# zdebruine/RcppML

Hardware: AMD Instinct MI355X
Metric: ALS updates/sec (cols solved/s), k=64 sparse NMF (higher is better)
Workload: dtype f32; 1 GPU; configs[1]: simulateNMF 20000x100000 (x1 GPUs, column shards) 1%-dense CSC, k=64, MSE, coordinate-descent NNLS (cd_maxit=100, cd_tol=1e-8), L1 row normalisation, loss every iteration; rows=20000, cols_per_gpu=100000, nnz_per_gpu=20054852, k=64, solver=cd, cd_variant=auto, parallelism=column-shard x1

## Files before the change

rcppml_amd/csrc/kernels_cd_mfma64.hip.h:

```cpp
#pragma once
#include "kernels.hip.h"

namespace rk {

template <class T> struct Vec4T;
template <> struct Vec4T<float> { typedef float4 type; };
template <> struct Vec4T<double> { typedef double4 type; };
template <int P> __device__ __forceinline__ unsigned bcast_row32(unsigned a) {
    if constexpr (P == 2) {
        return __builtin_amdgcn_permlane16_swap(a, a, false, false)[0];
    } else {
        const auto tu = __builtin_amdgcn_permlane16_swap(a, a, false, false);
        if constexpr (P == 0) {
            return __builtin_amdgcn_permlane32_swap(tu[0], tu[0], false, false)[0];
        } else {
            return __builtin_amdgcn_permlane32_swap(tu[1], tu[1], false, false)[0];
        }
    }
}
template <int P> __device__ __forceinline__ float bcast_row(float a) {
    return __uint_as_float(bcast_row32<P>(__float_as_uint(a)));
}
template <int P> __device__ __forceinline__ double bcast_row(double a) {
    const unsigned long long u = __double_as_longlong(a);
    const unsigned lo = bcast_row32<P>((unsigned)u), hi = bcast_row32<P>((unsigned)(u >> 32));
    return __longlong_as_double(((unsigned long long)hi << 32) | lo);
}

template <class T> struct CdStepOut64 { T a, nx; };
__device__ __forceinline__ float tmax(float a, float b) { return __builtin_fmaxf(a, b); }
__device__ __forceinline__ double tmax(double a, double b) { return __builtin_fmax(a, b); }

template <bool SIMPLE, class T>
__device__ __forceinline__ CdStepOut64<T> cd_step64(T b, T xo, T gd, T ginv, bool active, T l1_cd, T l2_cd, T lo, T hi) {
    CdStepOut64<T> o;
    if constexpr (SIMPLE) {
        const T diff = cd_quotient(b, gd, ginv);
        o.a = tmax(diff, -xo);
        o.nx = tmax(xo + diff, T(0));
    } else {
        T diff = cd_quotient(b, gd, ginv);
        diff -= l1_cd;
        diff = tfma(l2_cd, xo, diff);
        const T nv = xo + diff;
        const bool neg = nv < lo, up = nv > hi;
        T nx = neg ? lo : (up ? hi : nv);
        T a = neg ? lo - xo : (up ? hi - xo : diff);
        const bool on = active && (ginv > T(0));
        o.a = on ? a : T(0);
        o.nx = on ? nx : xo;
    }
    return o;
}

__device__ __forceinline__ f64x4 mfma16(double a, double b, f64x4 c) { return __builtin_amdgcn_mfma_f64_16x16x4f64(a, b, c, 0, 0, 0); }
typedef float f32x4 __attribute__((ext_vector_type(4)));
__device__ __forceinline__ f32x4 mfma16(float a, float b, f32x4 c) { return __builtin_amdgcn_mfma_f32_16x16x4f32(a, b, c, 0, 0, 0); }
template <class T> struct Acc4T;
template <> struct Acc4T<float> { typedef f32x4 type; };
template <> struct Acc4T<double> { typedef f64x4 type; };
__device__ __forceinline__ float fast_recip(float den) { return __builtin_amdgcn_rcpf(den); }
__device__ __forceinline__ double fast_recip(double den) {
    const double rc = __builtin_amdgcn_rcp(den);
    return __builtin_fma(__builtin_fma(-den, rc, 1.0), rc, rc);
}

template <class T, int NT, bool SIMPLE>
__global__ __launch_bounds__(256) __attribute__((amdgpu_waves_per_eu(NT <= 2 ? 4 : (NT <= 4 ? 2 : 1), 8)))
void cd_mfma64_kernel(const T* __restrict__ G , const T* __restrict__ B,
                      T* __restrict__ X, int k, int64_t ncols, T l1_pre, int warm, int zero_init, T l1_cd,
                      T l2_cd, int nonneg, int maxit, T tol, T ub_cd, T ub_post,
                      int* __restrict__ sweeps, const int* __restrict__ order, unsigned long long* __restrict__ stats) {
    typedef typename Vec4T<T>::type Tab4;
    typedef typename Acc4T<T>::type Acc4;
    constexpr int KP = 16 * NT;
    extern __shared__ __attribute__((aligned(16))) char smem_raw[];
    T* Gs = reinterpret_cast<T*>(smem_raw);
    Tab4* tab_s = reinterpret_cast<Tab4*>(Gs + KP * KP);
    [[maybe_unused]] T* gd_s = Gs + KP * KP + 4 * KP;
    {
        constexpr bool PERM = sizeof(T) == 4;
        auto gp = [&](int col, int row) { return (row < k && col < k) ? G[(int64_t)col * k + row] : (row == col ? T(1) : T(0)); };
        for (int e = threadIdx.x; e < KP * KP; e += blockDim.x) {
            const int qt = e >> 6, kk = (e >> 4) & 3, ps = e & 15;
            const int q = qt / NT, t = qt % NT;
            const int rl = PERM ? (ps >> 2) + 4 * (ps & 3) : ps;
            Gs[e] = -gp(4 * q + kk, 16 * t + rl);
        }
        for (int c = threadIdx.x; c < KP; c += blockDim.x) {
            const int gg = c & 3, qb = c & ~3;
            Tab4 v;
            const T gd = gp(c, c);
            v.x = gd > T(0) ? T(1) / gd : T(0);
            v.y = gg > 0 ? gp(qb + 0, c) : T(0);
            v.z = gg > 1 ? gp(qb + 1, c) : T(0);
            v.w = gg > 2 ? gp(qb + 2, c) : T(0);
            tab_s[c] = v;
            if constexpr (sizeof(T) == 8) gd_s[c] = gd > T(0) ? gd : T(0);
        }
    }
    __syncthreads();
    const int wave = threadIdx.x >> 6, lane = threadIdx.x & 63;
    const int g = lane >> 4, cl = lane & 15;
    const int64_t base = ((int64_t)blockIdx.x * (blockDim.x >> 6) + wave) * 16;
    if (base >= ncols) return;
    const int64_t slot = base + cl;
    const bool inb = slot < ncols;
    const int64_t j = (inb && order) ? order[slot] : slot;
    Acc4 acc[NT];
    T xr[NT][4];
    {
        const T* bj = B + j * (int64_t)k;
        const T* xj = X + j * (int64_t)k;
#pragma unroll
        for (int t = 0; t < NT; ++t)
#pragma unroll
            for (int v = 0; v < 4; ++v) {
                const int row = 16 * t + 4 * v + g;
                const bool ok = inb && row < k;
                T bv = ok ? bj[row] : T(0);
                if (ok && l1_pre != T(0)) bv -= l1_pre;
                acc[t][v] = bv;
                xr[t][v] = (ok && !zero_init) ? xj[row] : T(0);
            }
    }
    if (warm) {
#pragma unroll
        for (int t = 0; t < NT; ++t)
#pragma unroll
            for (int v = 0; v < 4; ++v) {
                const int q = 4 * t + v;
#pragma unroll
                for (int t2 = 0; t2 < NT; ++t2) {
                    const T av = Gs[((q * NT + t2) << 6) + lane];
                    acc[t2] = mfma16(av, xr[t][v], acc[t2]);
                }
            }
    }
    const T lo = nonneg ? T(0) : -INFINITY;
    const T hi = ub_cd > T(0) ? ub_cd : INFINITY;
    const bool check = tol > T(0);
    const T inv_k = T(1) / static_cast<T>(k);
    bool active = inb;
    int nsweep = 0;
    Tab4 tb_c = tab_s[g];
    [[maybe_unused]] T gd_c = T(0);
    if constexpr (sizeof(T) == 8) gd_c = gd_s[g];
    T av_c[NT];
#pragma unroll
    for (int t2 = 0; t2 < NT; ++t2) av_c[t2] = Gs[(t2 << 6) + lane];
    for (int it = 0; it < maxit; ++it) {
        if (!__any(active)) break;
        T tsum = T(0);
        nsweep += active ? 1 : 0;
#pragma unroll
        for (int t = 0; t < NT; ++t)
#pragma unroll
            for (int v = 0; v < 4; ++v) {
                constexpr int NQ = KP / 4;
                const int qn = (4 * t + v + 1) % NQ;
                const int tn = (v == 3 ? t + 1 : t) % NT;
                const Tab4 tb_n = tab_s[4 * qn + g];
                [[maybe_unused]] T gd_n = T(0);
                if constexpr (sizeof(T) == 8) gd_n = gd_s[4 * qn + g];
                T av_n[NT];
#pragma unroll
                for (int t2 = 0; t2 < NT; ++t2) av_n[t2] = Gs[((qn * NT + t2) << 6) + lane];
                const T b0 = acc[t][v];
                const T xo = xr[t][v];
                const T ginv = SIMPLE ? (active ? tb_c.x : T(0)) : tb_c.x;
                const CdStepOut64<T> s0 = cd_step64<SIMPLE, T>(b0, xo, gd_c, ginv, active, l1_cd, l2_cd, lo, hi);
                const T b1 = tfma(-tb_c.y, bcast_row<0>(s0.a), b0);
                const CdStepOut64<T> s1 = cd_step64<SIMPLE, T>(b1, xo, gd_c, ginv, active, l1_cd, l2_cd, lo, hi);
                const T b2 = tfma(-tb_c.z, bcast_row<1>(s1.a), b1);
                const CdStepOut64<T> s2 = cd_step64<SIMPLE, T>(b2, xo, gd_c, ginv, active, l1_cd, l2_cd, lo, hi);
                const T b3 = tfma(-tb_c.w, bcast_row<2>(s2.a), b2);
                const CdStepOut64<T> s3 = cd_step64<SIMPLE, T>(b3, xo, gd_c, ginv, active, l1_cd, l2_cd, lo, hi);
                xr[t][v] = s3.nx;
                tsum = tfma(tabs(s3.a), fast_recip(tabs(s3.nx) + T(1e-15)), tsum);
#pragma unroll
                for (int s = 0; s < NT; ++s) {
                    const int t2 = (tn + s) % NT;
                    acc[t2] = mfma16(av_c[t2], s3.a, acc[t2]);
                }
                tb_c = tb_n;
                gd_c = gd_n;
#pragma unroll
                for (int t2 = 0; t2 < NT; ++t2) av_c[t2] = av_n[t2];
                __builtin_amdgcn_sched_barrier(0);
            }
        T tot = tsum + __shfl_xor(tsum, 16, 64);
        tot += __shfl_xor(tot, 32, 64);
        active = active && !(check && tot * inv_k < tol);
    }
    if (inb) {
        T* xj = X + j * (int64_t)k;
#pragma unroll
        for (int t = 0; t < NT; ++t)
#pragma unroll
            for (int v = 0; v < 4; ++v) {
                const int row = 16 * t + 4 * v + g;
                if (row < k) {
                    T val = xr[t][v];
                    if (ub_post > T(0)) val = val < ub_post ? val : ub_post;
                    xj[row] = val;
                }
            }
        if (sweeps && g == 0) sweeps[j] = nsweep;
    }
    cd_stats_add(stats, (inb && g == 0) ? nsweep : 0, (inb && g == 0) ? 1 : 0);
}

}
```

rcppml_amd/csrc/solve_cd_impl.hip.h:

```cpp
#pragma once
#include <cmath>
#include "solve_common.hip.h"
#include "kernels_cd_mfma.hip.h"
#include "kernels_cd_mfma64.hip.h"
template <class T, int KP>
static void cd_lane_launch(rcppml_hip_ctx* c, const T* Gp, const T* invd, const T* B, T* X, int k,
                           int64_t ncols, T l1_pre, int warm, int zero_init, T l1_cd, T l2_cd, int nonneg,
                           int maxit, T tol, T ub_cd, T ub_post, int* sweeps, const int* order) {
    constexpr bool EXACT = std::is_same<T, double>::value;
    const int64_t nblk = (ncols + 63) / 64;
    hipLaunchKernelGGL((cd_lane_kernel<T, KP, EXACT>), dim3((unsigned)nblk), dim3(64), 0, c->stream, Gp, invd,
                       B, X, k, ncols, l1_pre, warm, zero_init, l1_cd, l2_cd, nonneg, maxit, tol, ub_cd, ub_post, sweeps, order, c->stats);
    HIPCHK(hipGetLastError());
}
template <class T, int KP, bool GLDS = true>
static void cd_wave_launch(rcppml_hip_ctx* c, const T* Gp, const T* invd, const T* B, T* X, int k,
                           int64_t ncols, T l1_pre, int warm, int zero_init, T l1_cd, T l2_cd, int nonneg,
                           int maxit, T tol, T ub_cd, T ub_post, int* sweeps, const int* order) {
    constexpr bool EXACT = std::is_same<T, double>::value;
    const size_t smem = GLDS ? (size_t)KP * KP * sizeof(T) : 0;
    auto kern = cd_wave_kernel<T, KP, EXACT, GLDS>;
    static DynSmemOnce once;
    once.ensure(reinterpret_cast<const void*>(kern), smem, c->device);
    int per_cu = (int)((160 * 1024) / (smem + 256));
    if (per_cu > 8) per_cu = 8;
    if (per_cu < 1) per_cu = 1;
    int64_t nblk = (int64_t)c->num_cu * per_cu;
    const int64_t need = (ncols + 3) / 4;
    if (nblk > need) nblk = need;
    if (nblk < 1) nblk = 1;
    hipLaunchKernelGGL(kern, dim3((unsigned)nblk), dim3(256), smem, c->stream, Gp, invd, B, X, k, ncols, l1_pre,
                       warm, zero_init, l1_cd, l2_cd, nonneg, maxit, tol, ub_cd, ub_post, sweeps, order, c->stats);
    HIPCHK(hipGetLastError());
}


template <class T, int KP, int LPC>
static void cd_group_launch(rcppml_hip_ctx* c, const T* Gp, const T* invd, const T* B, T* X, int k, int64_t ncols,
                            T l1_pre, int warm, int zero_init, T l1_cd, T l2_cd, int nonneg, int maxit, T tol, T ub_cd,
                            T ub_post, int* sweeps, const int* order) {
    constexpr bool EXACT = std::is_same<T, double>::value;
    const size_t smem = ((size_t)KP * KP + 2 * KP) * sizeof(T);
    auto kern = cd_group_kernel<T, KP, LPC, EXACT>;
    static DynSmemOnce once;
    once.ensure(reinterpret_cast<const void*>(kern), smem, c->device);
    const int64_t per_block = (int64_t)4 * (64 / LPC);
    const int64_t nblk = (ncols + per_block - 1) / per_block;
    hipLaunchKernelGGL(kern, dim3((unsigned)nblk), dim3(256), smem, c->stream, Gp, invd, B, X, k, ncols, l1_pre, warm,
                       zero_init, l1_cd, l2_cd, nonneg, maxit, tol, ub_cd, ub_post, sweeps, order, c->stats);
    HIPCHK(hipGetLastError());
}

template <int RT, int CT>
static void cd_mfma_launch(rcppml_hip_ctx* c, const float* G, const float* , const float* B, float* X, int k,
                           int64_t ncols, float l1_pre, int warm, int zero_init, float l1_cd, float l2_cd, int nonneg,
                           int maxit, float tol, float ub_cd, float ub_post, int* sweeps, const int* order) {
    size_t smem = cd_mfma_lds_bytes(RT);
    const int64_t per_block = 4 * 32 * CT;
    const int64_t nblk = (ncols + per_block - 1) / per_block;
    const bool simple = nonneg && ub_cd <= 0.f && l1_cd == 0.f && l2_cd == 0.f;
    {
        const double per_cu = (double)nblk / (double)(c->num_cu > 0 ? c->num_cu : 256);
        int cap = 0;
        if (per_cu > 1.0 && per_cu < 4.0 && per_cu - std::floor(per_cu) < 0.5) cap = (int)std::floor(per_cu);
        if (const char* e = exp_env("RCPPML_GPU_CD_CAP")) cap = atoi(e);
        if (cap > 0) {
            const size_t lds_cu = 160 * 1024;
            const size_t want = lds_cu / (size_t)(cap + 1) + 1024;
            if (want > smem && want <= lds_cu / (size_t)cap) smem = want;
        }
    }
    static DynSmemOnce once_simple, once_general;
    if (simple) once_simple.ensure(reinterpret_cast<const void*>(&cd_mfma_kernel<RT, CT, true>), smem, c->device);
    else once_general.ensure(reinterpret_cast<const void*>(&cd_mfma_kernel<RT, CT, false>), smem, c->device);
    if (simple)
        hipLaunchKernelGGL((cd_mfma_kernel<RT, CT, true>), dim3((unsigned)nblk), dim3(256), smem, c->stream, G, B, X,
                           k, ncols, l1_pre, warm, zero_init, l1_cd, l2_cd, nonneg, maxit, tol, ub_cd, ub_post, sweeps, order, c->stats);
    else
        hipLaunchKernelGGL((cd_mfma_kernel<RT, CT, false>), dim3((unsigned)nblk), dim3(256), smem, c->stream, G, B, X,
                           k, ncols, l1_pre, warm, zero_init, l1_cd, l2_cd, nonneg, maxit, tol, ub_cd, ub_post, sweeps, order, c->stats);
    HIPCHK(hipGetLastError());
}


void rcppml_cd_lmf_dispatch(rcppml_hip_ctx* c, const float* G, const float* B, float* X, int k, int64_t ncols, float l1_pre,
                            int warm, int zero_init, int maxit, float tol, float ub_post, int* sweeps, const int* order);

template <class T, int NT>
static void cd_mfma64_launch(rcppml_hip_ctx* c, const T* G, const T* , const T* B, T* X, int k,
                             int64_t ncols, T l1_pre, int warm, int zero_init, T l1_cd, T l2_cd, int nonneg,
                             int maxit, T tol, T ub_cd, T ub_post, int* sweeps, const int* order) {
    constexpr int KP = 16 * NT;
    const size_t smem = ((size_t)KP * KP + 4 * KP + (sizeof(T) == 8 ? KP : 0)) * sizeof(T);
    const int64_t nblk = (ncols + 63) / 64;
    const bool simple = nonneg && ub_cd <= T(0) && l1_cd == T(0) && l2_cd == T(0);
    static DynSmemOnce once_simple, once_general;
    if (simple) once_simple.ensure(reinterpret_cast<const void*>(&cd_mfma64_kernel<T, NT, true>), smem, c->device);
    else once_general.ensure(reinterpret_cast<const void*>(&cd_mfma64_kernel<T, NT, false>), smem, c->device);
    if (simple)
        hipLaunchKernelGGL((cd_mfma64_kernel<T, NT, true>), dim3((unsigned)nblk), dim3(256), smem, c->stream, G, B, X, k,
                           ncols, l1_pre, warm, zero_init, l1_cd, l2_cd, nonneg, maxit, tol, ub_cd, ub_post, sweeps, order, c->stats);
    else
        hipLaunchKernelGGL((cd_mfma64_kernel<T, NT, false>), dim3((unsigned)nblk), dim3(256), smem, c->stream, G, B, X, k,
                           ncols, l1_pre, warm, zero_init, l1_cd, l2_cd, nonneg, maxit, tol, ub_cd, ub_post, sweeps, order, c->stats);
    HIPCHK(hipGetLastError());
}

template <class T>
static int pick_lpc(int KP) {
    const int ev = 16 / (int)sizeof(T);
    const char* e = exp_env("RCPPML_GPU_CD_LPC");
    int lpc = e ? atoi(e) : (std::is_same<T, float>::value ? KP / 32 : KP / 16);
    if (lpc < 1) lpc = 1;
    if (lpc > 4) lpc = 4;
    while (lpc < 4 && KP / lpc > 32) lpc *= 2;
    while (lpc > 1 && (KP / lpc) % ev != 0) lpc /= 2;
    return lpc;
}

template <class T>
static void solve_cd_impl(rcppml_hip_ctx* c, const T* G, const T* B, T* X, int k, int64_t ncols, T l1_pre,
                          int warm, int zero_init, T l1_cd, T l2_cd, int nonneg, int maxit, T tol, T ub_cd,
                          T ub_post, int variant, int* sweeps, const int* order) {
    if (ncols <= 0) return;
    if (k < 1 || k > 256) throw std::runtime_error("solve_cd: k must be in [1,256]");
    if (k > 128) {
        T *Gp, *invd;
        pad_impl<T>(c, G, k, 256, &Gp, &invd);
        cd_wave_launch<T, 256, false>(c, Gp, invd, B, X, k, ncols, l1_pre, warm, zero_init, l1_cd, l2_cd, nonneg, maxit, tol, ub_cd,
                                      ub_post, sweeps, order);
        return;
    }
    int KP = solve_kp(k);
    const bool lmf_ok = std::is_same<T, float>::value && k <= 64 && nonneg && ub_cd <= T(0) && l1_cd == T(0) && l2_cd == T(0) && maxit >= 1;
    if (variant == RCPPML_CD_LMF && !lmf_ok) variant = RCPPML_CD_AUTO;
    if (variant == RCPPML_CD_AUTO && lmf_ok && k <= 32 && ncols >= (int64_t)256 * c->num_cu && !c->opt_cd_no_lmf &&
        !exp_env("RCPPML_GPU_CD_VARIANT"))
        variant = RCPPML_CD_LMF;
    if (variant == RCPPML_CD_LMF) {
        if constexpr (std::is_same<T, float>::value)
            rcppml_cd_lmf_dispatch(c, G, B, X, k, ncols, l1_pre, warm, zero_init, maxit, tol, ub_post, sweeps, order);
        return;
    }
    if (variant == RCPPML_CD_AUTO && k <= 64 && nonneg && ub_cd <= T(0) && l1_cd == T(0) && l2_cd == T(0) && maxit >= 1 &&
        ncols <= (int64_t)6 * (c->num_cu > 0 ? c->num_cu : 256) && !exp_env("RCPPML_GPU_CD_VARIANT")) {
        const unsigned nblk = (unsigned)((ncols + 3) / 4);
        if (k <= 16)
            hipLaunchKernelGGL((cd_wave_static_kernel<T, 16>), dim3(nblk), dim3(256), 0, c->stream, G, B, X, k, ncols, l1_pre, warm, zero_init,
                               maxit, tol, ub_post, sweeps, c->stats);
        else if (k <= 32)
            hipLaunchKernelGGL((cd_wave_static_kernel<T, 32>), dim3(nblk), dim3(256), 0, c->stream, G, B, X, k, ncols, l1_pre, warm, zero_init,
                               maxit, tol, ub_post, sweeps, c->stats);
        else
            hipLaunchKernelGGL((cd_wave_static_kernel<T, 64>), dim3(nblk), dim3(256), 0, c->stream, G, B, X, k, ncols, l1_pre, warm, zero_init,
                               maxit, tol, ub_post, sweeps, c->stats);
        HIPCHK(hipGetLastError());
        return;
    }
    if (variant == RCPPML_CD_AUTO) {
        const char* e = exp_env("RCPPML_GPU_CD_VARIANT");
        if (e && !strcmp(e, "lane")) variant = RCPPML_CD_LANE;
        else if (e && !strcmp(e, "wave")) variant = RCPPML_CD_WAVE;
        else if (e && !strcmp(e, "group")) variant = RCPPML_CD_GROUP;
        else if (e && !strcmp(e, "mfma")) variant = RCPPML_CD_MFMA;
        else if (e && !strcmp(e, "mfma16")) variant = RCPPML_CD_MFMA16;
        else variant = RCPPML_CD_MFMA;
        if (variant == RCPPML_CD_MFMA && std::is_same<T, float>::value && k <= 64 && !e) {
            static int small16 = -1;
            if (small16 < 0) small16 = exp_flag("RCPPML_GPU_CD_SMALL16", "0") ? 0 : 1;
            if (small16 && (ncols + 31) / 32 < (int64_t)4 * c->num_cu) variant = RCPPML_CD_MFMA16;
        }
    }
    if (variant == RCPPML_CD_MFMA && !std::is_same<T, float>::value) variant = RCPPML_CD_MFMA16;
    if (variant == RCPPML_CD_MFMA16 && k > 64 && std::is_same<T, float>::value) variant = RCPPML_CD_MFMA;
    if (variant == RCPPML_CD_MFMA) KP = 32 * ((k + 31) / 32);
    if (variant == RCPPML_CD_MFMA16) KP = 16 * ((k + 15) / 16);
    const int lane_max = std::is_same<T, float>::value ? 64 : 32;
    if (variant == RCPPML_CD_LANE && KP > lane_max) variant = RCPPML_CD_GROUP;
    if (variant != RCPPML_CD_LANE && variant != RCPPML_CD_WAVE && variant != RCPPML_CD_MFMA && variant != RCPPML_CD_MFMA16) variant = RCPPML_CD_GROUP;
    if (variant == RCPPML_CD_WAVE && KP < 64) KP = 64;
    T *Gp = const_cast<T*>(G), *invd = nullptr;
    if (variant != RCPPML_CD_MFMA && variant != RCPPML_CD_MFMA16) pad_impl<T>(c, G, k, KP, &Gp, &invd);
#define CD_ARGS c, Gp, invd, B, X, k, ncols, l1_pre, warm, zero_init, l1_cd, l2_cd, nonneg, maxit, tol, ub_cd, ub_post, sweeps, order
    if (variant == RCPPML_CD_LANE) {
        switch (KP) {
            case 16: cd_lane_launch<T, 16>(CD_ARGS); break;
            case 32: cd_lane_launch<T, 32>(CD_ARGS); break;
            default:
                if constexpr (std::is_same<T, float>::value) cd_lane_launch<T, 64>(CD_ARGS);
                break;
        }
    } else if (variant == RCPPML_CD_MFMA) {
        if constexpr (std::is_same<T, float>::value) {
            switch (KP) {
                case 32: cd_mfma_launch<1, 1>(CD_ARGS); break;
                case 64: cd_mfma_launch<2, 1>(CD_ARGS); break;
                case 96: cd_mfma_launch<3, 1>(CD_ARGS); break;
                default: cd_mfma_launch<4, 1>(CD_ARGS); break;
            }
        }
    } else if (variant == RCPPML_CD_MFMA16) {
        switch (KP) {
            case 16: cd_mfma64_launch<T, 1>(CD_ARGS); break;
            case 32: cd_mfma64_launch<T, 2>(CD_ARGS); break;
            case 48: cd_mfma64_launch<T, 3>(CD_ARGS); break;
            case 64: cd_mfma64_launch<T, 4>(CD_ARGS); break;
            default:
                if constexpr (std::is_same<T, double>::value) {
                    switch (KP) {
                        case 80: cd_mfma64_launch<T, 5>(CD_ARGS); break;
                        case 96: cd_mfma64_launch<T, 6>(CD_ARGS); break;
                        case 112: cd_mfma64_launch<T, 7>(CD_ARGS); break;
                        default: cd_mfma64_launch<T, 8>(CD_ARGS); break;
                    }
                } else cd_mfma64_launch<T, 4>(CD_ARGS);
                break;
        }
    } else if (variant == RCPPML_CD_GROUP) {
        const int lpc = pick_lpc<T>(KP);
#define GROUP_CASE(K_, L_) if (KP == K_ && lpc == L_) { cd_group_launch<T, K_, L_>(CD_ARGS); launched = true; }
        bool launched = false;
        GROUP_CASE(16, 1) GROUP_CASE(16, 2) GROUP_CASE(16, 4)
        GROUP_CASE(32, 1) GROUP_CASE(32, 2) GROUP_CASE(32, 4)
        GROUP_CASE(64, 2) GROUP_CASE(64, 4)
        GROUP_CASE(128, 4)
#undef GROUP_CASE
        if (!launched) throw std::runtime_error("solve_cd: no lane-group configuration for this rank");
    } else {
        if (KP == 64) cd_wave_launch<T, 64>(CD_ARGS);
        else cd_wave_launch<T, 128>(CD_ARGS);
    }
#undef CD_ARGS
}
```

Measured before the change: 105.3 million cols/s.

## Pack per-quad Gram operands into vector LDS loads and trim CD inner loop

For f32, the Gram image in LDS is repacked so that the NT A-operands a lane needs for one quad sit contiguously and are fetched with a single vector load, replacing NT scalar LDS reads. The permlane row broadcasts now pass a prior value as the discarded operand, and a no-check max helper replaces fmax in the simple step. In the simple path, inactive columns no longer mask ginv each step; their accumulators are zeroed once when they converge instead. NT==3 pads to a 4-wide vector, which uses more LDS.

```diff
diff --git a/rcppml_amd/csrc/kernels_cd_mfma64.hip.h b/rcppml_amd/csrc/kernels_cd_mfma64.hip.h
--- a/rcppml_amd/csrc/kernels_cd_mfma64.hip.h
+++ b/rcppml_amd/csrc/kernels_cd_mfma64.hip.h
@@ -1,42 +1,44 @@
 #pragma once
 #include "kernels.hip.h"
+#include "kernels_cd_mfma.hip.h"
 
 namespace rk {
 
 template <class T> struct Vec4T;
 template <> struct Vec4T<float> { typedef float4 type; };
 template <> struct Vec4T<double> { typedef double4 type; };
-template <int P> __device__ __forceinline__ unsigned bcast_row32(unsigned a) {
+template <int P> __device__ __forceinline__ unsigned bcast_row32(unsigned a, unsigned junk) {
     if constexpr (P == 2) {
-        return __builtin_amdgcn_permlane16_swap(a, a, false, false)[0];
+        return __builtin_amdgcn_permlane16_swap(junk, a, false, false)[0];
+    } else if constexpr (P == 1) {
+        const auto tu = __builtin_amdgcn_permlane16_swap(a, a, false, false);
+        return __builtin_amdgcn_permlane32_swap(junk, tu[1], false, false)[0];
     } else {
         const auto tu = __builtin_amdgcn_permlane16_swap(a, a, false, false);
-        if constexpr (P == 0) {
-            return __builtin_amdgcn_permlane32_swap(tu[0], tu[0], false, false)[0];
-        } else {
-            return __builtin_amdgcn_permlane32_swap(tu[1], tu[1], false, false)[0];
-        }
-    }
-}
-template <int P> __device__ __forceinline__ float bcast_row(float a) {
-    return __uint_as_float(bcast_row32<P>(__float_as_uint(a)));
-}
-template <int P> __device__ __forceinline__ double bcast_row(double a) {
-    const unsigned long long u = __double_as_longlong(a);
-    const unsigned lo = bcast_row32<P>((unsigned)u), hi = bcast_row32<P>((unsigned)(u >> 32));
+        return __builtin_amdgcn_permlane32_swap(tu[0], tu[0], false, false)[0];
+    }
+}
+template <int P> __device__ __forceinline__ float bcast_row(float a, float junk) {
+    return __uint_as_float(bcast_row32<P>(__float_as_uint(a), __float_as_uint(junk)));
+}
+template <int P> __device__ __forceinline__ double bcast_row(double a, double junk) {
+    const unsigned long long u = __double_as_longlong(a), ju = __double_as_longlong(junk);
+    const unsigned lo = bcast_row32<P>((unsigned)u, (unsigned)ju), hi = bcast_row32<P>((unsigned)(u >> 32), (unsigned)(ju >> 32));
     return __longlong_as_double(((unsigned long long)hi << 32) | lo);
 }
 
 template <class T> struct CdStepOut64 { T a, nx; };
 __device__ __forceinline__ float tmax(float a, float b) { return __builtin_fmaxf(a, b); }
 __device__ __forceinline__ double tmax(double a, double b) { return __builtin_fmax(a, b); }
+__device__ __forceinline__ float cd_max64(float a, float b, float inf) { return cd_max_nc(a, b, inf); }
+__device__ __forceinline__ double cd_max64(double a, double b, double ) { return __builtin_fmax(a, b); }
 
 template <bool SIMPLE, class T>
 __device__ __forceinline__ CdStepOut64<T> cd_step64(T b, T xo, T gd, T ginv, bool active, T l1_cd, T l2_cd, T lo, T hi) {
     CdStepOut64<T> o;
     if constexpr (SIMPLE) {
         const T diff = cd_quotient(b, gd, ginv);
-        o.a = tmax(diff, -xo);
+        o.a = cd_max64(diff, -xo, hi);
         o.nx = tmax(xo + diff, T(0));
     } else {
         T diff = cd_quotient(b, gd, ginv);
@@ -65,6 +67,14 @@
     return __builtin_fma(__builtin_fma(-den, rc, 1.0), rc, rc);
 }
 
+template <int W> struct CdPk64 { typedef float type __attribute__((ext_vector_type(W))); };
+template <> struct CdPk64<1> { typedef float type; };
+template <class T> __host__ __device__ constexpr size_t cd_mfma64_lds_bytes(int NT) {
+    const size_t KP = 16 * (size_t)NT;
+    return sizeof(T) == 8 ? (KP * KP + 4 * KP + KP) * sizeof(T)
+                          : ((KP / 4) * 64 * (size_t)(NT == 3 ? 4 : NT) + 4 * KP) * sizeof(T);
+}
+
 template <class T, int NT, bool SIMPLE>
 __global__ __launch_bounds__(256) __attribute__((amdgpu_waves_per_eu(NT <= 2 ? 4 : (NT <= 4 ? 2 : 1), 8)))
 void cd_mfma64_kernel(const T* __restrict__ G , const T* __restrict__ B,
@@ -73,19 +83,32 @@
                       int* __restrict__ sweeps, const int* __restrict__ order, unsigned long long* __restrict__ stats) {
     typedef typename Vec4T<T>::type Tab4;
     typedef typename Acc4T<T>::type Acc4;
-    constexpr int KP = 16 * NT;
+    constexpr int KP = 16 * NT, NQ = KP / 4;
+    constexpr bool PACK = sizeof(T) == 4;
+    constexpr int PW = NT == 3 ? 4 : NT;
+    typedef typename CdPk64<PW>::type Pk;
+    constexpr int IMG = PACK ? NQ * 64 * PW : KP * KP;
     extern __shared__ __attribute__((aligned(16))) char smem_raw[];
     T* Gs = reinterpret_cast<T*>(smem_raw);
-    Tab4* tab_s = reinterpret_cast<Tab4*>(Gs + KP * KP);
-    [[maybe_unused]] T* gd_s = Gs + KP * KP + 4 * KP;
+    [[maybe_unused]] Pk* pk_s = reinterpret_cast<Pk*>(smem_raw);
+    Tab4* tab_s = reinterpret_cast<Tab4*>(Gs + IMG);
+    [[maybe_unused]] T* gd_s = Gs + IMG + 4 * KP;
     {
-        constexpr bool PERM = sizeof(T) == 4;
         auto gp = [&](int col, int row) { return (row < k && col < k) ? G[(int64_t)col * k + row] : (row == col ? T(1) : T(0)); };
-        for (int e = threadIdx.x; e < KP * KP; e += blockDim.x) {
-            const int qt = e >> 6, kk = (e >> 4) & 3, ps = e & 15;
-            const int q = qt / NT, t = qt % NT;
-            const int rl = PERM ? (ps >> 2) + 4 * (ps & 3) : ps;
-            Gs[e] = -gp(4 * q + kk, 16 * t + rl);
+        if constexpr (PACK) {
+            for (int e = threadIdx.x; e < NQ * 64; e += blockDim.x) {
+                const int q = e >> 6, kk = (e >> 4) & 3, ps = e & 15;
+                const int rl = (ps >> 2) + 4 * (ps & 3);
+                T* dst = Gs + (size_t)e * PW;
+#pragma unroll
+                for (int t = 0; t < PW; ++t) dst[t] = t < NT ? -gp(4 * q + kk, 16 * t + rl) : T(0);
+            }
+        } else {
+            for (int e = threadIdx.x; e < KP * KP; e += blockDim.x) {
+                const int qt = e >> 6, kk = (e >> 4) & 3, ps = e & 15;
+                const int q = qt / NT, t = qt % NT;
+                Gs[e] = -gp(4 * q + kk, 16 * t + ps);
+            }
         }
         for (int c = threadIdx.x; c < KP; c += blockDim.x) {
             const int gg = c & 3, qb = c & ~3;
@@ -124,17 +147,30 @@
                 xr[t][v] = (ok && !zero_init) ? xj[row] : T(0);
             }
     }
+    struct QuadOps { T av[NT]; };
+    auto load_quad = [&](int q) {
+        QuadOps o;
+        if constexpr (PACK) {
+            const Pk p = pk_s[q * 64 + lane];
+            if constexpr (NT == 1) o.av[0] = p;
+            else {
+#pragma unroll
+                for (int t2 = 0; t2 < NT; ++t2) o.av[t2] = p[t2];
+            }
+        } else {
+#pragma unroll
+            for (int t2 = 0; t2 < NT; ++t2) o.av[t2] = Gs[((q * NT + t2) << 6) + lane];
+        }
+        return o;
+    };
     if (warm) {
 #pragma unroll
         for (int t = 0; t < NT; ++t)
 #pragma unroll
             for (int v = 0; v < 4; ++v) {
-                const int q = 4 * t + v;
-#pragma unroll
-                for (int t2 = 0; t2 < NT; ++t2) {
-                    const T av = Gs[((q * NT + t2) << 6) + lane];
-                    acc[t2] = mfma16(av, xr[t][v], acc[t2]);
-                }
+                const QuadOps wo = load_quad(4 * t + v);
+#pragma unroll
+                for (int t2 = 0; t2 < NT; ++t2) acc[t2] = mfma16(wo.av[t2], xr[t][v], acc[t2]);
             }
     }
     const T lo = nonneg ? T(0) : -INFINITY;
@@ -146,9 +182,7 @@
     Tab4 tb_c = tab_s[g];
     [[maybe_unused]] T gd_c = T(0);
     if constexpr (sizeof(T) == 8) gd_c = gd_s[g];
-    T av_c[NT];
-#pragma unroll
-    for (int t2 = 0; t2 < NT; ++t2) av_c[t2] = Gs[(t2 << 6) + lane];
+    QuadOps op_c = load_quad(0);
     for (int it = 0; it < maxit; ++it) {
         if (!__any(active)) break;
         T tsum = T(0);
@@ -157,41 +191,49 @@
         for (int t = 0; t < NT; ++t)
 #pragma unroll
             for (int v = 0; v < 4; ++v) {
-                constexpr int NQ = KP / 4;
                 const int qn = (4 * t + v + 1) % NQ;
                 const int tn = (v == 3 ? t + 1 : t) % NT;
+                const T b0 = acc[t][v];
+                const T xo = xr[t][v];
+                const T ginv = tb_c.x;
+                const QuadOps op_n = load_quad(qn);
                 const Tab4 tb_n = tab_s[4 * qn + g];
                 [[maybe_unused]] T gd_n = T(0);
                 if constexpr (sizeof(T) == 8) gd_n = gd_s[4 * qn + g];
-                T av_n[NT];
-#pragma unroll
-                for (int t2 = 0; t2 < NT; ++t2) av_n[t2] = Gs[((qn * NT + t2) << 6) + lane];
-                const T b0 = acc[t][v];
-                const T xo = xr[t][v];
-                const T ginv = SIMPLE ? (active ? tb_c.x : T(0)) : tb_c.x;
                 const CdStepOut64<T> s0 = cd_step64<SIMPLE, T>(b0, xo, gd_c, ginv, active, l1_cd, l2_cd, lo, hi);
-                const T b1 = tfma(-tb_c.y, bcast_row<0>(s0.a), b0);
+                const T c0 = bcast_row<0>(s0.a, T(0));
+                const T b1 = tfma(-tb_c.y, c0, b0);
                 const CdStepOut64<T> s1 = cd_step64<SIMPLE, T>(b1, xo, gd_c, ginv, active, l1_cd, l2_cd, lo, hi);
-                const T b2 = tfma(-tb_c.z, bcast_row<1>(s1.a), b1);
+                const T c1 = bcast_row<1>(s1.a, c0);
+                const T b2 = tfma(-tb_c.z, c1, b1);
                 const CdStepOut64<T> s2 = cd_step64<SIMPLE, T>(b2, xo, gd_c, ginv, active, l1_cd, l2_cd, lo, hi);
-                const T b3 = tfma(-tb_c.w, bcast_row<2>(s2.a), b2);
+                const T c2 = bcast_row<2>(s2.a, c1);
+                const T b3 = tfma(-tb_c.w, c2, b2);
                 const CdStepOut64<T> s3 = cd_step64<SIMPLE, T>(b3, xo, gd_c, ginv, active, l1_cd, l2_cd, lo, hi);
                 xr[t][v] = s3.nx;
                 tsum = tfma(tabs(s3.a), fast_recip(tabs(s3.nx) + T(1e-15)), tsum);
 #pragma unroll
                 for (int s = 0; s < NT; ++s) {
                     const int t2 = (tn + s) % NT;
-                    acc[t2] = mfma16(av_c[t2], s3.a, acc[t2]);
+                    acc[t2] = mfma16(op_c.av[t2], s3.a, acc[t2]);
                 }
                 tb_c = tb_n;
                 gd_c = gd_n;
-#pragma unroll
-                for (int t2 = 0; t2 < NT; ++t2) av_c[t2] = av_n[t2];
+                op_c = op_n;
                 __builtin_amdgcn_sched_barrier(0);
             }
         T tot = tsum + __shfl_xor(tsum, 16, 64);
         tot += __shfl_xor(tot, 32, 64);
-        active = active && !(check && tot * inv_k < tol);
+        const bool now = active && !(check && tot * inv_k < tol);
+        if constexpr (SIMPLE) {
+            if (__any(active && !now)) {
+#pragma unroll
+                for (int t = 0; t < NT; ++t)
+#pragma unroll
+                    for (int v = 0; v < 4; ++v) acc[t][v] = now ? acc[t][v] : T(0);
+            }
+        }
+        active = now;
     }
     if (inb) {
         T* xj = X + j * (int64_t)k;
diff --git a/rcppml_amd/csrc/solve_cd_impl.hip.h b/rcppml_amd/csrc/solve_cd_impl.hip.h
--- a/rcppml_amd/csrc/solve_cd_impl.hip.h
+++ b/rcppml_amd/csrc/solve_cd_impl.hip.h
@@ -90,8 +90,7 @@
 static void cd_mfma64_launch(rcppml_hip_ctx* c, const T* G, const T* , const T* B, T* X, int k,
                              int64_t ncols, T l1_pre, int warm, int zero_init, T l1_cd, T l2_cd, int nonneg,
                              int maxit, T tol, T ub_cd, T ub_post, int* sweeps, const int* order) {
-    constexpr int KP = 16 * NT;
-    const size_t smem = ((size_t)KP * KP + 4 * KP + (sizeof(T) == 8 ? KP : 0)) * sizeof(T);
+    const size_t smem = cd_mfma64_lds_bytes<T>(NT);
     const int64_t nblk = (ncols + 63) / 64;
     const bool simple = nonneg && ub_cd <= T(0) && l1_cd == T(0) && l2_cd == T(0);
     static DynSmemOnce once_simple, once_general;
```

Result: no change. 106.2 million cols/s, median of 6 (+0.8%).
